# douban/fast_tffm

Measured on AMD Instinct MI355X. Metric: examples/sec (whole node), Criteo-shaped FM k=64, higher is better.
Workload: dtype fp32; 1 GPU; model=FM k=64, fp32 table + adagrad, hashed vocab 125000000 (125000000/GPU), global_batch=131072, seq_len=39, parallelism=single, lookahead=2, pool=16, rccl_world=1, comm_bytes_per_rank=0

## Files before the change

### fast_tffm_amd/csrc/hip/fm_common.h

```cpp
#pragma once
#include <hip/hip_runtime.h>
#include <hip/hip_bf16.h>
#include <cstdint>

namespace fm {

constexpr int kWave = 64;
constexpr int kBlock = 256;
constexpr int kWavesPerBlock = kBlock / kWave;

constexpr int kChunkSegMask = (1 << 30) - 1;
constexpr int kChunkFirst = 1 << 30;
constexpr unsigned kChunkSingle = 1u << 31;

constexpr int kDevErrSort = 1;
__device__ int g_fm_dev_error = 0;

enum LossType : int { kLossNone = 0, kLossMse = 1, kLossLogistic = 2 };
enum OptType : int { kOptAdagrad = 0, kOptFtrl = 1, kOptSgd = 2 };
enum DType : int { kF32 = 0, kBF16 = 1, kFP8 = 2 };

struct fp8e4m3 { uint8_t bits; };
constexpr float kFp8Max = 448.f;

// ... 237 lines not shown
  if constexpr (StateBf16<TV>::v) {
    uint16_t* p = reinterpret_cast<uint16_t*>(s) + off;
    uint32_t b[EPL];
#pragma unroll
    for (int k = 0; k < EPL; k += 4) {
      if (seed) {
        const uint32_t r = sr_hash(seed, row, col + (uint32_t)k);
#pragma unroll
        for (int i = 0; i < 4; ++i) b[k + i] = f32_to_bf16_bits_sr(o[k + i], sr_word(r, i));
      } else {
#pragma unroll
        for (int i = 0; i < 4; ++i) b[k + i] = f32_to_bf16_bits(o[k + i]);
      }
    }
    if constexpr (EPL % 8 == 0) {
#pragma unroll
      for (int k = 0; k < EPL; k += 8)
        *reinterpret_cast<uint4*>(p + k) = make_uint4(b[k] | (b[k + 1] << 16), b[k + 2] | (b[k + 3] << 16),
                                                      b[k + 4] | (b[k + 5] << 16), b[k + 6] | (b[k + 7] << 16));
    } else {
#pragma unroll
      for (int k = 0; k < EPL; k += 4)
        *reinterpret_cast<uint2*>(p + k) = make_uint2(b[k] | (b[k + 1] << 16), b[k + 2] | (b[k + 3] << 16));
    }
  } else {
    float* p = reinterpret_cast<float*>(s) + off;
#pragma unroll
    for (int k = 0; k < EPL; k += 4) *reinterpret_cast<float4*>(p + k) = make_float4(o[k], o[k + 1], o[k + 2], o[k + 3]);
  }
}
constexpr uint32_t kSrSalt0 = 0x68e31da4u, kSrSalt1 = 0xb5297a4du;

template <typename TV>
__device__ inline float row_scale(const float* w, long long row, long long w_stride) {
  if constexpr (Frag<TV>::kScaled) return w[row * w_stride + 1];
  return 1.f;
}

constexpr int kFp8Norm = 2;
template <int LPR>
__device__ inline float fp8_norm2(int u, float s, bool tact) {
  float q[4];
  Frag<fp8e4m3>::cvt(u, q);
  float p = tact ? __fmaf_rn(q[0], q[0], __fmaf_rn(q[1], q[1], __fmaf_rn(q[2], q[2], q[3] * q[3]))) : 0.f;
  p = group_sum<LPR>(p);
  return p * (s * s);
}

template <int LPR, typename TV>
__device__ inline void store_row(TV* lane_ptr, const float (&o)[Frag<TV>::N], float* w, long long row,
                                 long long w_stride, int t, bool tact, uint32_t sr_seed = 0) {
  using F = Frag<TV>;
  const uint32_t col = (uint32_t)(t * F::N);
  if constexpr (F::kScaled) {
    float m = 0.f;
#pragma unroll
    for (int k = 0; k < F::N; ++k) m = fmaxf(m, fabsf(o[k]));
    m = group_max<LPR>(m);
    const float s = fp8_row_scale(m);
    const float inv = 1.f / s;
    float q[F::N];
#pragma unroll
    for (int k = 0; k < F::N; ++k) q[k] = fminf(fmaxf(o[k] * inv, -kFp8Max), kFp8Max);
    int u = 0;
    if (tact) u = sr_seed ? F::store_sr(lane_ptr, q, sr_seed, (uint32_t)row, col) : F::store(lane_ptr, q);
    const float n2 = fp8_norm2<LPR>(u, s, tact);
    if (t == 0) {
      w[row * w_stride + 1] = s;
      w[row * w_stride + kFp8Norm] = n2;
    }
  } else {
    if (tact) {
      if (sr_seed) F::store_sr(lane_ptr, o, sr_seed, (uint32_t)row, col);
      else F::store(lane_ptr, o);
    }
  }
}

template <int LPR>
__device__ inline void store_row_fp8x8(fp8e4m3* lane_ptr, const float (&o)[8], float* w, long long row,
                                       long long w_stride, int t, bool tact, uint32_t sr_seed) {
  using F = Frag<fp8e4m3>;
  float m = 0.f;
#pragma unroll
  for (int k = 0; k < 8; ++k) m = fmaxf(m, fabsf(o[k]));
  m = group_max<LPR>(m);
  const float s = fp8_row_scale(m);
  const float inv = 1.f / s;
  float qa[4], qb[4];
#pragma unroll
  for (int k = 0; k < 4; ++k) {
    qa[k] = fminf(fmaxf(o[k] * inv, -kFp8Max), kFp8Max);
    qb[k] = fminf(fmaxf(o[k + 4] * inv, -kFp8Max), kFp8Max);
  }
  const uint32_t col = (uint32_t)(t * 8);
  int ua = 0, ub = 0;
  if (tact) {
    ua = sr_seed ? F::pack_sr(qa, sr_seed, (uint32_t)row, col) : F::pack(qa);
    ub = sr_seed ? F::pack_sr(qb, sr_seed, (uint32_t)row, col + 4) : F::pack(qb);
    *reinterpret_cast<uint2*>(lane_ptr) = make_uint2((uint32_t)ua, (uint32_t)ub);
  }
  float pa[4], pb[4];
  F::cvt(ua, pa);
  F::cvt(ub, pb);
  float na = tact ? __fmaf_rn(pa[0], pa[0], __fmaf_rn(pa[1], pa[1], __fmaf_rn(pa[2], pa[2], pa[3] * pa[3]))) : 0.f;
  float nb = tact ? __fmaf_rn(pb[0], pb[0], __fmaf_rn(pb[1], pb[1], __fmaf_rn(pb[2], pb[2], pb[3] * pb[3]))) : 0.f;
  na = group_sum<LPR>(na);
  nb = group_sum<LPR>(nb);
  const float n2 = (na + nb) * (s * s);
  if (t == 0) {
    w[row * w_stride + 1] = s;
    w[row * w_stride + kFp8Norm] = n2;
  }
}

#ifndef FM_FP8_WIDE
#define FM_FP8_WIDE 1
#endif

template <typename TV, int EPL>
__device__ inline void frag_load(const TV* p, float (&o)[EPL]) {
  if constexpr (EPL == Frag<TV>::N) {
    Frag<TV>::load(p, o);
  } else {
    static_assert(std::is_same<TV, fp8e4m3>::value && EPL == 8, "wide rows: fp8, 8 values per lane");
    const uint2 u = *reinterpret_cast<const uint2*>(p);
    float lo[4], hi[4];
    Frag<TV>::cvt((int)u.x, lo);
    Frag<TV>::cvt((int)u.y, hi);
#pragma unroll
    for (int k = 0; k < 4; ++k) {
      o[k] = lo[k];
      o[k + 4] = hi[k];
    }
  }
}
template <int LPR, typename TV, int EPL>
__device__ inline void store_row_e(TV* lane_ptr, const float (&o)[EPL], float* w, long long row, long long w_stride,
                                   int t, bool tact, uint32_t sr) {
  if constexpr (EPL == Frag<TV>::N) store_row<LPR, TV>(lane_ptr, o, w, row, w_stride, t, tact, sr);
  else store_row_fp8x8<LPR>(lane_ptr, o, w, row, w_stride, t, tact, sr);
}

__device__ inline uint32_t sr_step_seed(const int* counter) {
  return counter ? (sr_hash((uint32_t)*counter, 0x5bd1e995u, 0x1b873593u) | 1u) : 0u;
}

template <int LPR>
__device__ inline float across_groups_sum(float v) {
#pragma unroll
  for (int o = LPR; o < kWave; o <<= 1) v += __shfl_xor(v, o, kWave);
  return v;
}

__device__ inline float softplus_neg_abs(float p) {
  return log1pf(__expf(-fabsf(p)));
}

__device__ inline float sigmoidf(float p) { return 1.f / (1.f + __expf(-p)); }

struct OptParams {
  int type;
  float lr;
  float l1, l2;
  float beta;
};

struct SelfRows {
  int u0, u1;
  long long base;
  const int* keys;
  const int* excl;
  const void* v; long long v_stride;
  float* w; long long w_stride;
  __device__ inline bool has(int u) const { return u >= u0 && u < u1; }
  __device__ inline bool exclusive(int u) const { return excl == nullptr || excl[u - u0] != 0; }
  __device__ inline long long row(int u) const { return (long long)keys[u] - base; }
};

__device__ inline void opt_step(const OptParams& o, float g, float& p, float& s0, float& s1) {
  if (o.type == kOptAdagrad) {
    s0 += g * g;
    p -= o.lr * g * rsqrtf(s0);
  } else if (o.type == kOptFtrl) {
    const float n_new = s0 + g * g;
    const float sq_old = sqrtf(s0), sq_new = sqrtf(n_new);
    s1 += g - (sq_new - sq_old) / o.lr * p;
    s0 = n_new;
    const float quad = (o.beta + sq_new) / o.lr + 2.f * o.l2;
    p = fabsf(s1) > o.l1 ? (copysignf(o.l1, s1) - s1) / quad : 0.f;
  } else {
    p -= o.lr * g;
  }
}

template <typename TV>
__device__ inline void opt_step_tv(const OptParams& o, float g, float& p, float& s0, float& s1) {
  if constexpr (FM_FP8_FAST_EPI && StateBf16<TV>::v) {
    if (o.type == kOptFtrl) {
      const float ilr = __builtin_amdgcn_rcpf(o.lr);
      const float n_new = __builtin_fmaf(g, g, s0);
      const float sq_old = __builtin_amdgcn_sqrtf(s0), sq_new = __builtin_amdgcn_sqrtf(n_new);
      s1 += __builtin_fmaf(-((sq_new - sq_old) * ilr), p, g);
      s0 = n_new;
      const float quad = __builtin_fmaf(o.beta + sq_new, ilr, 2.f * o.l2);
      p = fabsf(s1) > o.l1 ? (copysignf(o.l1, s1) - s1) * __builtin_amdgcn_rcpf(quad) : 0.f;
      return;
    }
    if (o.type == kOptAdagrad) {
      s0 = __builtin_fmaf(g, g, s0);
      p = __builtin_fmaf(-(o.lr * g), __builtin_amdgcn_rsqf(s0), p);
      return;
    }
  }
  opt_step(o, g, p, s0, s1);
}

template <typename TV, int N>
__device__ inline void opt_step_row(const OptParams& o, const float (&g)[N], float (&p)[N], float (&s0)[N],
                                    float (&s1)[N]) {
  if (o.type == kOptFtrl) {
    OptParams f = o;
    f.type = kOptFtrl;
#pragma unroll
    for (int k = 0; k < N; ++k) opt_step_tv<TV>(f, g[k], p[k], s0[k], s1[k]);
  } else if (o.type == kOptAdagrad) {
    OptParams f = o;
    f.type = kOptAdagrad;
#pragma unroll
    for (int k = 0; k < N; ++k) opt_step_tv<TV>(f, g[k], p[k], s0[k], s1[k]);
  } else {
#pragma unroll
    for (int k = 0; k < N; ++k) p[k] -= o.lr * g[k];
  }
}

inline int next_pow2(int x) { int p = 1; while (p < x) p <<= 1; return p; }

inline int lanes_per_row(int Kp, int dtype) {
  const int epl = 4;
  return next_pow2((Kp + epl - 1) / epl);
}

inline int lds_for_wg_per_cu(int n, int static_lds) {
  static const int cu_lds = [] {
    int dev = 0, v = 0;
    (void)hipGetDevice(&dev);
    if (hipDeviceGetAttribute(&v, hipDeviceAttributeMaxSharedMemoryPerMultiprocessor, dev) != hipSuccess || v <= 0)
      v = 160 * 1024;
    return v;
  }();
  const int per = cu_lds / (n + 1) + 1024 - static_lds;
  return per > 0 && (per + static_lds) * n <= cu_lds ? per : 0;
}

inline int fill_grid(long long work_groups, int groups_per_block, int cap = 8192) {
  long long blocks = (work_groups + groups_per_block - 1) / groups_per_block;
  if (blocks < 1) blocks = 1;
  if (blocks > cap) blocks = cap;
  return (int)blocks;
}

#define FM_DISPATCH_LPR(LPR_VAL, KERNEL, TV, GRID, SHM, STREAM, ARGS)                                   \
  switch (LPR_VAL) {                                                                                     \
    case 1: hipLaunchKernelGGL((KERNEL<1, TV>), dim3(GRID), dim3(kBlock), SHM, STREAM, ARGS); break;     \
    case 2: hipLaunchKernelGGL((KERNEL<2, TV>), dim3(GRID), dim3(kBlock), SHM, STREAM, ARGS); break;     \
    case 4: hipLaunchKernelGGL((KERNEL<4, TV>), dim3(GRID), dim3(kBlock), SHM, STREAM, ARGS); break;     \
    case 8: hipLaunchKernelGGL((KERNEL<8, TV>), dim3(GRID), dim3(kBlock), SHM, STREAM, ARGS); break;     \
    case 16: hipLaunchKernelGGL((KERNEL<16, TV>), dim3(GRID), dim3(kBlock), SHM, STREAM, ARGS); break;   \
    case 32: hipLaunchKernelGGL((KERNEL<32, TV>), dim3(GRID), dim3(kBlock), SHM, STREAM, ARGS); break;   \
    case 64: hipLaunchKernelGGL((KERNEL<64, TV>), dim3(GRID), dim3(kBlock), SHM, STREAM, ARGS); break;   \
    default: return -1;                                                                                  \
  }

#define FM_DISPATCH_WIDE_LPR(LPR_VAL, KERNEL, TV, GRID, SHM, STREAM, ARGS)                              \
  switch (LPR_VAL) {                                                                                     \
    case 4: hipLaunchKernelGGL((KERNEL<4, TV>), dim3(GRID), dim3(kBlock), SHM, STREAM, ARGS); break;     \
    case 8: hipLaunchKernelGGL((KERNEL<8, TV>), dim3(GRID), dim3(kBlock), SHM, STREAM, ARGS); break;     \
    case 16: hipLaunchKernelGGL((KERNEL<16, TV>), dim3(GRID), dim3(kBlock), SHM, STREAM, ARGS); break;   \
    case 32: hipLaunchKernelGGL((KERNEL<32, TV>), dim3(GRID), dim3(kBlock), SHM, STREAM, ARGS); break;   \
    case 64: hipLaunchKernelGGL((KERNEL<64, TV>), dim3(GRID), dim3(kBlock), SHM, STREAM, ARGS); break;   \
    default: return -1;                                                                                  \
  }

#define FM_DISPATCH_TV(DTYPE, M, LPR_VAL, KERNEL, GRID, SHM, STREAM, ARGS)   \
  if ((DTYPE) == kBF16) {                                                   \
    M(LPR_VAL, KERNEL, __hip_bfloat16, GRID, SHM, STREAM, ARGS)             \
  } else if ((DTYPE) == kFP8) {                                             \
    M(LPR_VAL, KERNEL, fp8e4m3, GRID, SHM, STREAM, ARGS)                    \
  } else {                                                                  \
    M(LPR_VAL, KERNEL, float, GRID, SHM, STREAM, ARGS)                      \
  }
#define FM_DISPATCH_WIDE(DTYPE, LPR_VAL, KERNEL, GRID, SHM, STREAM, ARGS) \
  FM_DISPATCH_TV(DTYPE, FM_DISPATCH_WIDE_LPR, LPR_VAL, KERNEL, GRID, SHM, STREAM, ARGS)
#define FM_DISPATCH_SHM(DTYPE, LPR_VAL, KERNEL, GRID, SHM, STREAM, ARGS) \
  FM_DISPATCH_TV(DTYPE, FM_DISPATCH_LPR, LPR_VAL, KERNEL, GRID, SHM, STREAM, ARGS)
#define FM_DISPATCH(DTYPE, LPR_VAL, KERNEL, GRID, STREAM, ARGS) \
  FM_DISPATCH_SHM(DTYPE, LPR_VAL, KERNEL, GRID, 0, STREAM, ARGS)

}
```

### fast_tffm_amd/csrc/hip/fm_fwd.hip

```cpp
#include "fm_common.h"

namespace fm {

struct FwdArgs {
  int B;
  const int* offsets;
  const int* rows;
  const float* vals;
  const void* v;
  long long v_stride;
  const float* w;
  long long w_stride;
  int Kp;
  const float* labels;
  const float* weights;
  int loss_type;
  float grad_scale;
  float* pred;
  void* r1;
  float* dpred;
  float* loss_partial;
  float* reg_partial;
  const float* bias;
  SelfRows self;
  const int* seg_idx;
  const int* seg_keys;
  int seg_shift;
  int max_feats;
};

__device__ inline int seg_lookup(const FwdArgs& a, int k) {
  const int b = (int)((uint32_t)k >> a.seg_shift);
  int s = a.seg_idx[b];
  const int e = a.seg_idx[b + 1];
  while (s + 1 < e && a.seg_keys[s] != k) ++s;
  return s;
}

#ifndef FM_FWD_PREFETCH
#define FM_FWD_PREFETCH 1
#endif
#ifndef FM_FWD_SPECIALIZE
#define FM_FWD_SPECIALIZE 1
#endif
constexpr int kSelfBit = (int)0x80000000u;
template <int G>
struct FwdUnroll {
  static constexpr int v = ((40 + G - 1) / G) > 12 ? 12 : ((40 + G - 1) / G);
};

template <int LPR, typename TV>
constexpr int fwd_min_waves() {
  return LPR >= 32 ? 4 : 1;
}
#ifndef FM_FWD_LOCAL_W16
#define FM_FWD_LOCAL_W16 7
#endif
#ifndef FM_FWD_UNR16
#define FM_FWD_UNR16 2
#endif
#ifndef FM_FWD_LOCAL_W32
#define FM_FWD_LOCAL_W32 4
#endif
#ifndef FM_FWD_UNR32
#define FM_FWD_UNR32 12
#endif
#ifndef FM_FWD_LOCAL_W32_FP8
#define FM_FWD_LOCAL_W32_FP8 7
#endif
#ifndef FM_FWD_UNR32_FP8
#define FM_FWD_UNR32_FP8 4
#endif
#ifndef FM_FWD_LOCAL_W4
#define FM_FWD_LOCAL_W4 4
#endif
#ifndef FM_FWD_UNR4
#define FM_FWD_UNR4 5
#endif
#ifndef FM_FWD_UNR16_SH
#define FM_FWD_UNR16_SH 10
#endif
#ifndef FM_FWD_SH_W16
#define FM_FWD_SH_W16 4
#endif
template <typename TV>
constexpr bool fwd_is_bf16() { return std::is_same<TV, __hip_bfloat16>::value; }
template <int LPR, typename TV, bool SH = false>
constexpr int fwd_local_min_waves() {
  return LPR == 4 && fwd_is_bf16<TV>() && FM_FWD_LOCAL_W4 > 0 ? FM_FWD_LOCAL_W4
         : LPR == 16 ? (SH && !Frag<TV>::kScaled ? FM_FWD_SH_W16 : FM_FWD_LOCAL_W16)
         : LPR == 32 ? (Frag<TV>::kScaled ? FM_FWD_LOCAL_W32_FP8 : FM_FWD_LOCAL_W32)
                     : fwd_min_waves<LPR, TV>();
}
template <int LPR, typename TV, bool SH = false>
constexpr int fwd_unroll() {
  return LPR == 16 && SH && !Frag<TV>::kScaled ? FM_FWD_UNR16_SH
         : LPR == 4 && fwd_is_bf16<TV>() && FM_FWD_UNR4 > 0 ? FM_FWD_UNR4
         : LPR == 16 ? FM_FWD_UNR16
         : LPR == 32 ? (Frag<TV>::kScaled ? FM_FWD_UNR32_FP8 : FM_FWD_UNR32)
                     : FwdUnroll<kWave / LPR>::v;
}

template <int LPR, typename TV, bool SH>
__device__ __forceinline__ void fwd_body(const FwdArgs& a) {
  using F = Frag<TV>;
  constexpr int EPL = F::N;
  constexpr int G = kWave / LPR;
  constexpr int UNR = fwd_unroll<LPR, TV, SH>();
  constexpr bool kRaw = F::kScaled;
  constexpr bool kNorm = F::kScaled;
  const int lane = threadIdx.x & (kWave - 1);
  const int g = lane / LPR, t = lane % LPR;
  const int nv = a.Kp / EPL;
  const bool tact = t < nv;
  const int tE = tact ? t : nv - 1;
  const float tmask = tact ? 1.f : 0.f;
  const uint32_t coff = (uint32_t)(tE * EPL * (int)sizeof(TV));
  const char* vbytes = reinterpret_cast<const char*>(a.v) + coff;
  const uint32_t vsb = (uint32_t)(a.v_stride * (long long)sizeof(TV));
  const bool self_on = SH && a.self.u1 > a.self.u0;
  const uint32_t tsb = self_on ? (uint32_t)(a.self.v_stride * (long long)sizeof(TV)) : vsb;
  const uint64_t wbase = reinterpret_cast<uint64_t>(a.v) + coff;
  const uint64_t sbase = self_on ? reinterpret_cast<uint64_t>(a.self.v) + coff : wbase;
  const int wave = blockIdx.x * kWavesPerBlock + (threadIdx.x >> 6);
  const int nwaves = gridDim.x * kWavesPerBlock;
  const bool want_reg = a.reg_partial != nullptr;
  const bool self_key = SH && self_on && a.seg_idx != nullptr;
  const int self_kmin = self_key ? a.self.keys[a.self.u0] : 0;
  const int self_kmax = self_key ? a.self.keys[a.self.u1 - 1] : -1;
  const int wv = threadIdx.x >> 6;

  float loss_acc = 0.f, regv_acc = 0.f, regw_acc = 0.f;
  constexpr bool kPrefetch = FM_FWD_PREFETCH;
  auto pairs = [&](int base, int m, int& row, float& x) {
    row = 0;
    x = 0.f;
    if (lane < m) {
      row = a.rows[base + lane];
      x = a.vals ? a.vals[base + lane] : 1.f;
    }
  };
  int s = 0, e = 0, sn = 0, en = 0;
  int p_row = 0;
  float p_x = 0.f;
  if (wave < a.B) {
    s = a.offsets[wave];
    e = a.offsets[wave + 1];
    if (kPrefetch) pairs(s, min(kWave, e - s), p_row, p_x);
  }
  if (wave + nwaves < a.B) {
    sn = a.offsets[wave + nwaves];
    en = a.offsets[wave + nwaves + 1];
  }
  for (int i = wave; i < a.B; i += nwaves) {
    int n_row = 0;
    float n_x = 0.f;
    if (kPrefetch) pairs(sn, i + nwaves < a.B ? min(kWave, en - sn) : 0, n_row, n_x);
    int snn = 0, enn = 0;
    if (i + 2 * nwaves < a.B) {
      snn = a.offsets[i + 2 * nwaves];
      enn = a.offsets[i + 2 * nwaves + 1];
    }
    float y_pre = 0.f, wt_pre = 1.f;
    if (kPrefetch && a.loss_type != kLossNone && lane == 0) {
      y_pre = a.labels[i];
      if (a.weights) wt_pre = a.weights[i];
    }
    float s1[EPL], s2[EPL];
#pragma unroll
    for (int k = 0; k < EPL; ++k) { s1[k] = 0.f; s2[k] = 0.f; }
    float lin = 0.f, rv = 0.f, rw = 0.f;
    float s2n = 0.f;
    for (int base = s; base < e; base += kWave) {
      const int m = min(kWave, e - base);
      int my_row = 0;
      float my_x = 0.f, my_w = 0.f, my_s = 1.f, my_n2 = 0.f;
      uint32_t my_t = 0;
      if (kPrefetch && base == s) {
        my_row = p_row;
        my_x = p_x;
      } else {
        pairs(base, m, my_row, my_x);
      }
      if constexpr (!SH) {
        if (lane < m) {
          if constexpr (kNorm) {
            const float4 wr = *reinterpret_cast<const float4*>(a.w + (uint64_t)(uint32_t)my_row * 4u);
            my_w = wr.x;
            my_s = wr.y;
            my_n2 = wr.z;
          } else {
            my_w = a.w[(long long)my_row * a.w_stride];
          }
        }
      } else {
        if (lane < m) {
          const int key = my_row;
          const bool own_key = self_key && key >= self_kmin && key <= self_kmax;
          if (a.seg_idx && !own_key) my_row = seg_lookup(a, key);
          const bool own = own_key || (self_on && !self_key && a.self.has(my_row));
          const long long r = own ? (own_key ? (long long)key - a.self.base : a.self.row(my_row)) : my_row;
          my_t = (uint32_t)r | (own ? 0x80000000u : 0u);
          const uint64_t wp = reinterpret_cast<uint64_t>(own ? a.self.w + r * a.self.w_stride : a.w + r * a.w_stride);
          if constexpr (kNorm) {
            const gf4 wr = *gptr<gf4>(wp);
            my_w = wr.x;
            my_s = wr.y;
            my_n2 = wr.z;
          } else {
            my_w = *gptr<float>(wp);
          }
        }
        const uint32_t t0 = (uint32_t)__builtin_amdgcn_readfirstlane((int)my_t);
        if (lane >= m) my_t = t0;
      }

      for (int q = 0; q < m; q += G * UNR) {
        float fr[UNR][EPL], fx[UNR], fs[UNR];
        int fraw[kRaw ? UNR : 1];
#pragma unroll
        for (int u = 0; u < UNR; ++u) {
          const int f = q + u * G + g;
          const int fb = (f & (kWave - 1)) << 2;
          const float x = __int_as_float(__builtin_amdgcn_ds_bpermute(fb, __float_as_int(my_x)));
          fx[u] = f < m ? x : 0.f;
          if constexpr (SH) {
            const uint32_t tr = (uint32_t)__builtin_amdgcn_ds_bpermute(fb, (int)my_t);
            const bool own = (tr >> 31) != 0;
            const uint64_t pr = (own ? sbase : wbase) + (uint64_t)(tr & 0x7fffffffu) * (own ? tsb : vsb);
            if constexpr (kRaw) fraw[u] = *gptr<int>(pr);
            else F::load_g(pr, fr[u]);
          } else {
            const int row = __builtin_amdgcn_ds_bpermute(fb, my_row);
            const char* rp = vbytes + (uint64_t)(uint32_t)row * vsb;
            if constexpr (kRaw) fraw[u] = *reinterpret_cast<const int*>(rp);
            else F::load(reinterpret_cast<const TV*>(rp), fr[u]);
          }
          if constexpr (F::kScaled) fs[u] = __int_as_float(__builtin_amdgcn_ds_bpermute(fb, __float_as_int(my_s)));
        }
#pragma unroll
        for (int u = 0; u < UNR; ++u) {
          float (&fv)[EPL] = fr[u];
          if constexpr (kRaw) F::cvt_scaled(fraw[u], fs[u], fv);
          const float xm = fx[u] * tmask;
#pragma unroll
          for (int k = 0; k < EPL; ++k) {
            const float xv = xm * fv[k];
            s1[k] += xv;
            if constexpr (!kNorm) s2[k] += xv * xv;
          }
          if (!kNorm && want_reg) {
            const float ok = (q + u * G + g) < m ? 1.f : 0.f;
#pragma unroll
            for (int k = 0; k < EPL; ++k) rv += ok * tmask * fv[k] * fv[k];
          }
        }
      }
      lin += my_x * my_w;
      if (want_reg) rw += my_w * my_w;
      if constexpr (kNorm) {
        s2n += my_x * my_x * my_n2;
        if (want_reg && lane < m) rv += my_n2;
      }
    }
    float part = 0.f;
#pragma unroll
    for (int k = 0; k < EPL; ++k) {
      s1[k] = across_groups_sum<LPR>(s1[k]);
      s2[k] = across_groups_sum<LPR>(s2[k]);
      part += s1[k] * s1[k] - s2[k];
    }
    part = group_sum<LPR>(part);
    if constexpr (kNorm) part -= group_sum<kWave>(s2n);
    lin = group_sum<kWave>(lin);
    const float pred = lin + 0.5f * part + (a.bias ? a.bias[0] : 0.f);
    if (a.r1 != nullptr && g == 0 && tact) store_r1<TV, EPL>(a.r1, (long long)i * a.Kp + t * EPL, s1);
    if (want_reg) {
      rv = group_sum<kWave>(rv);
      rw = group_sum<kWave>(rw);
      regv_acc += rv;
      regw_acc += rw;
    }
    float l = 0.f, d = 0.f;
    if (a.loss_type != kLossNone && lane == 0) {
      const float y = kPrefetch ? y_pre : a.labels[i];
      const float wt = kPrefetch ? wt_pre : (a.weights ? a.weights[i] : 1.f);
      if (a.loss_type == kLossMse) {
        const float diff = pred - y;
        l = wt * diff * diff;
        d = 2.f * wt * diff;
      } else {
        l = wt * (fmaxf(pred, 0.f) - pred * y + softplus_neg_abs(pred));
        d = wt * (sigmoidf(pred) - y);
      }
    }
    if (lane == 0) {
      a.pred[i] = pred;
      if (a.loss_type != kLossNone) {
        loss_acc += l;
        if (a.dpred) a.dpred[i] = d * a.grad_scale;
      }
    }
    s = sn; e = en; sn = snn; en = enn;
    p_row = n_row; p_x = n_x;
  }
  if (a.loss_partial == nullptr && a.reg_partial == nullptr) return;
  __shared__ float red[3][kWavesPerBlock];
  if (lane == 0) {
    red[0][wv] = loss_acc;
    red[1][wv] = regv_acc;
    red[2][wv] = regw_acc;
  }
  __syncthreads();
  if (threadIdx.x == 0) {
    float l = 0.f, r0 = 0.f, r1v = 0.f;
    for (int k = 0; k < kWavesPerBlock; ++k) { l += red[0][k]; r0 += red[1][k]; r1v += red[2][k]; }
    if (a.loss_partial) a.loss_partial[blockIdx.x] = l;
    if (a.reg_partial) { a.reg_partial[2 * blockIdx.x] = r0; a.reg_partial[2 * blockIdx.x + 1] = r1v; }
  }
}

template <int LPR, typename TV>
__global__ __launch_bounds__(kBlock) __attribute__((amdgpu_waves_per_eu(fwd_local_min_waves<LPR, TV>())))
void fm_fwd_kernel(FwdArgs a) {
  fwd_body<LPR, TV, false>(a);
}

template <int LPR, typename TV>
__global__ __launch_bounds__(kBlock) __attribute__((amdgpu_waves_per_eu(fwd_local_min_waves<LPR, TV, true>())))
void fm_fwd_shard_kernel(FwdArgs a) {
  fwd_body<LPR, TV, true>(a);
}

#ifndef FM_WITH_MFMA
#define FM_WITH_MFMA 0
#endif
#if FM_WITH_MFMA
#include "fm_fwd_mfma.hip"
#endif

__global__ __launch_bounds__(kBlock) void csr_rows_kernel(int B, const int* offsets, int* ex_of_occ, int slot_bits) {
  const int lane = threadIdx.x & (kWave - 1);
  const int ngroups = (B + kWave - 1) / kWave;
  const int nwaves = gridDim.x * kWavesPerBlock;
  for (int g = blockIdx.x * kWavesPerBlock + (threadIdx.x >> 6); g < ngroups; g += nwaves) {
    const int i0 = g * kWave;
    const int n = min(kWave, B - i0);
    const int o = offsets[i0 + min(lane, n)];
    const int s = __shfl(o, 0);
    const int e = offsets[i0 + n];
    for (int base = s; base < e; base += kWave) {
      const int p = base + lane;
      int k = 0;
#pragma unroll
      for (int step = kWave / 2; step > 0; step >>= 1) {
        const int c = k + step;
        if (__shfl(o, c) <= p) k = c;
      }
      const int ok = __shfl(o, k);
      if (p < e) {
        const int ex = i0 + k;
        ex_of_occ[p] = slot_bits > 0 ? (ex << slot_bits) | (p - ok) : ex;
      }
    }
  }
}

static bool g_fwd_mfma = FM_WITH_MFMA;
bool fwd_mfma_enabled() { return g_fwd_mfma; }
void set_fwd_mfma(bool on) { g_fwd_mfma = FM_WITH_MFMA && on; }

int fwd_grid(int B) { return fill_grid(B, kWavesPerBlock, 4096); }

int launch_fwd(const FwdArgs& a, int dtype, int grid, hipStream_t st) {
  if (a.B <= 0) return 0;
  const int lpr = lanes_per_row(a.Kp, dtype);
  if (dtype == kFP8) {
    auto aligned = [](const float* w, long long ws) { return ((uintptr_t)w & 15) == 0 && ws % 4 == 0; };
    if (!aligned(a.w, a.w_stride) || (a.self.u1 > a.self.u0 && !aligned(a.self.w, a.self.w_stride))) return -7;
  }
  const bool table_rows = dtype != kFP8 || a.w_stride == 4;
#if FM_WITH_MFMA
  if (fwd_mfma_enabled() && dtype == kFP8 && a.Kp == kMfRowB && a.v_stride == kMfRowB && !a.vals && table_rows &&
      a.self.u1 <= a.self.u0 && !a.seg_idx && a.max_feats > 0 && a.max_feats * kMfT <= kMfMaxRows) {
    hipLaunchKernelGGL(fm_fwd_mfma_fp8_kernel, dim3(grid), dim3(kBlock), 0, st, a);
    return (int)hipGetLastError();
  }
#endif

  if (a.self.u1 > a.self.u0 || a.seg_idx || !FM_FWD_SPECIALIZE || !table_rows) {
    FM_DISPATCH(dtype, lpr, fm_fwd_shard_kernel, grid, st, a);
  } else {
    FM_DISPATCH(dtype, lpr, fm_fwd_kernel, grid, st, a);
  }
  return (int)hipGetLastError();
}

int launch_csr_rows(int B, const int* offsets, int* ex_of_occ, int slot_bits, hipStream_t st) {
  if (B <= 0) return 0;
  hipLaunchKernelGGL(csr_rows_kernel, dim3(fill_grid((B + kWave - 1) / kWave, kWavesPerBlock, 4096)), dim3(kBlock), 0, st, B,
                     offsets, ex_of_occ, slot_bits);
  return (int)hipGetLastError();
}

}
```

### fast_tffm_amd/csrc/hip/module.hip

```cpp
#include <pybind11/pybind11.h>
#include <pybind11/stl.h>
#include <stdexcept>
#include <string>
#include "fm_common.h"

namespace py = pybind11;

#ifndef FM_HIP_MODULE
#define FM_HIP_MODULE _fm_hip
#endif
using u64 = std::uintptr_t;

#include "fm_bwd.hip"
#include "fm_fwd.hip"
#include "fm_explain.hip"
#include "fm_topk.hip"
#include "dedup.hip"
#include "metric_common.hip"
#include "auc.hip"
#include "isotonic.hip"
#include "gauc.hip"
#include "shard.hip"
#include "init.hip"
#include "ckpt.hip"
#include "parse.hip"
#include "batch_gather.hip"
#include "feeder.hip"

namespace {

template <typename T> T* P(u64 p) { return reinterpret_cast<T*>(p); }
hipStream_t S(u64 s) { return reinterpret_cast<hipStream_t>(s); }

void check(int code, const char* what) {
  if (code != 0) {
    std::string msg = std::string(what) + " failed: ";
    msg += code > 0 ? hipGetErrorString(static_cast<hipError_t>(code)) : ("code " + std::to_string(code));
    throw std::runtime_error(msg);
  }
}

fm::SelfRows self_rows(const std::vector<long long>& f) {
  fm::SelfRows r{};
  if (f.empty()) return r;
  if (f.size() != 9) throw std::invalid_argument("self_rows: [u0, u1, base, keys, excl, v, v_stride, w, w_stride]");
  if (f[1] > f[0] && (!f[3] || !f[5] || !f[7])) throw std::runtime_error("self rows need keys and the table");
  r.u0 = (int)f[0]; r.u1 = (int)(f[1] > f[0] ? f[1] : f[0]); r.base = f[2];
  r.keys = P<const int>((u64)f[3]); r.excl = P<const int>((u64)f[4]);
  r.v = P<const void>((u64)f[5]); r.v_stride = f[6]; r.w = P<float>((u64)f[7]); r.w_stride = f[8];
  return r;
}

fm::OptParams opt_params(int type, float lr, float l1, float l2, float beta) {
  fm::OptParams o;
  o.type = type; o.lr = lr; o.l1 = l1; o.l2 = l2; o.beta = beta;
  return o;
}

}

#ifndef FM_BUILD_HASH
#define FM_BUILD_HASH "unhashed"
#endif
extern "C" __attribute__((used, visibility("default"))) const char fm_build_hash_marker[] = "FMBUILDHASH:" FM_BUILD_HASH;

PYBIND11_MODULE(FM_HIP_MODULE, m) {
  m.doc() = "gfx950 HIP kernels for fast_tffm_amd (FM forward/backward/optimizer, dedup, sharding)";
  m.attr("ARCH") = "gfx950";
  m.attr("BUILD_HASH") = FM_BUILD_HASH;
  m.attr("MAX_CH") = fm::kMaxCH;

  m.def("fwd_grid", &fm::fwd_grid, py::arg("B"));
  m.def("fwd_mfma_enabled", &fm::fwd_mfma_enabled);
  m.def("set_fwd_mfma", &fm::set_fwd_mfma, py::arg("on"));
#if FM_MF_PROF
  m.def("mf_prof", [] {
    unsigned long long h[8] = {};
    hipDeviceSynchronize();
    hipMemcpyFromSymbol(h, HIP_SYMBOL(fm::g_mf_prof), sizeof(h));
    const unsigned long long z[8] = {};
    hipMemcpyToSymbol(HIP_SYMBOL(fm::g_mf_prof), z, sizeof(z));
    return std::vector<unsigned long long>(h, h + 8);
  });
#endif
  m.def("lanes_per_row", &fm::lanes_per_row, py::arg("Kp"), py::arg("dtype"));

  m.def(
      "fwd",
      [](int B, u64 offsets, u64 rows, u64 vals, u64 v, long long v_stride, u64 w, long long w_stride, int Kp,
         int dtype, u64 labels, u64 weights, int loss_type, float grad_scale, u64 pred, u64 r1, u64 dpred,
         u64 loss_partial, u64 reg_partial, int grid, u64 stream, u64 bias, const std::vector<long long>& self,
         u64 seg_idx, u64 seg_keys, int seg_shift, int max_feats) {
        fm::FwdArgs a{};
        a.max_feats = max_feats;
        a.seg_idx = P<const int>(seg_idx); a.seg_keys = P<const int>(seg_keys); a.seg_shift = seg_shift;
        if (a.seg_idx && (!a.seg_keys || seg_shift < 0 || seg_shift > 31))
          throw std::invalid_argument("fm_fwd: segment lookup needs the sorted keys and a shift in [0, 31]");
        a.self = self_rows(self);
        a.B = B; a.offsets = P<const int>(offsets); a.rows = P<const int>(rows);
        a.vals = P<const float>(vals); a.v = P<const void>(v); a.v_stride = v_stride;
        a.w = P<const float>(w); a.w_stride = w_stride; a.Kp = Kp;
        a.labels = P<const float>(labels); a.weights = P<const float>(weights);
        a.loss_type = loss_type; a.grad_scale = grad_scale; a.pred = P<float>(pred);
        a.r1 = P<void>(r1); a.dpred = P<float>(dpred); a.loss_partial = P<float>(loss_partial);
        a.reg_partial = P<float>(reg_partial); a.bias = P<const float>(bias);
        check(fm::launch_fwd(a, dtype, grid, S(stream)), "fm_fwd");
      },
      py::arg("B"), py::arg("offsets"), py::arg("rows"), py::arg("vals"), py::arg("v"), py::arg("v_stride"),
      py::arg("w"), py::arg("w_stride"), py::arg("Kp"), py::arg("dtype"), py::arg("labels"), py::arg("weights"),
      py::arg("loss_type"), py::arg("grad_scale"), py::arg("pred"), py::arg("r1"), py::arg("dpred"),
      py::arg("loss_partial"), py::arg("reg_partial"), py::arg("grid"), py::arg("stream"), py::arg("bias") = 0,
      py::arg("self_rows") = std::vector<long long>{}, py::arg("seg_idx") = 0, py::arg("seg_keys") = 0,
      py::arg("seg_shift") = 0, py::arg("max_feats") = -1);

  m.def(
      "explain",
      [](int B, u64 offsets, u64 rows, u64 vals, u64 v, long long v_stride, u64 w, long long w_stride, int Kp,
         int dtype, u64 bias, u64 contrib, u64 pred, u64 stream) {
        fm::ExplainArgs a{};
        a.B = B; a.offsets = P<const int>(offsets); a.rows = P<const int>(rows); a.vals = P<const float>(vals);
        a.v = P<const void>(v); a.v_stride = v_stride; a.w = P<const float>(w); a.w_stride = w_stride; a.Kp = Kp;
        a.bias = P<const float>(bias); a.contrib = P<float>(contrib); a.pred = P<float>(pred);
        check(fm::launch_explain(a, dtype, S(stream)), "fm_explain");
      },
      py::arg("B"), py::arg("offsets"), py::arg("rows"), py::arg("vals"), py::arg("v"), py::arg("v_stride"),
      py::arg("w"), py::arg("w_stride"), py::arg("Kp"), py::arg("dtype"), py::arg("bias"), py::arg("contrib"),
      py::arg("pred"), py::arg("stream"));
  m.def(
      "importance",
      [](int U, u64 contrib, u64 perm, u64 seg_start, u64 count, u64 sum_abs, u64 sum, u64 stream) {
        fm::ImportanceArgs a{};
        a.U = U; a.contrib = P<const float>(contrib); a.perm = P<const int>(perm);
        a.seg_start = P<const int>(seg_start); a.count = P<int>(count); a.sum_abs = P<double>(sum_abs);
        a.sum = P<double>(sum);
        check(fm::launch_importance(a, S(stream)), "fm_importance");
      },
      py::arg("U"), py::arg("contrib"), py::arg("perm"), py::arg("seg_start"), py::arg("count"), py::arg("sum_abs"),
      py::arg("sum"), py::arg("stream"));

  m.def(
      "topk_plan",
      [](long long nq, long long nc, int k) {
        const fm::topk::Plan p = fm::topk::plan(nq, nc, k);
        return py::make_tuple(p.slab, p.parts);
      },
      py::arg("nq"), py::arg("nc"), py::arg("k"));
  m.def("topk_workspace_bytes", &fm::topk_workspace_bytes, py::arg("nq"), py::arg("nc"), py::arg("k"));
  m.def(
      "topk",
      [](long long nq, long long nc, int Kp, int k, u64 q, long long q_stride, u64 c, long long c_stride, u64 qb,
         u64 cb, u64 ws, size_t ws_bytes, u64 idx, u64 score, u64 stream) {
        if ((long long)ws_bytes < fm::topk_workspace_bytes(nq, nc, k)) throw std::runtime_error("topk: workspace too small");
        fm::TopkArgs a{};
        a.nq = nq; a.nc = nc; a.Kp = Kp; a.k = k; a.Q = P<const float>(q); a.q_stride = q_stride;
        a.C = P<const float>(c); a.c_stride = c_stride; a.qb = P<const float>(qb); a.cb = P<const float>(cb);
        a.ws = P<unsigned long long>(ws); a.idx = P<int>(idx); a.score = P<float>(score);
        check(fm::launch_topk(a, S(stream)), "fm_topk");
      },
      py::arg("nq"), py::arg("nc"), py::arg("Kp"), py::arg("k"), py::arg("q"), py::arg("q_stride"), py::arg("c"),
      py::arg("c_stride"), py::arg("qb"), py::arg("cb"), py::arg("ws"), py::arg("ws_bytes"), py::arg("idx"),
      py::arg("score"), py::arg("stream"));

  m.def(
      "seg_index",
      [](int n_max, u64 uniq, u64 counts, int shift, int nb, u64 idx, u64 stream) {
        check(fm::launch_seg_index(n_max, P<const uint32_t>(uniq), P<const int>(counts), shift, nb, P<int>(idx),
                                   S(stream)),
              "seg_index");
      },
      py::arg("n_max"), py::arg("uniq"), py::arg("counts"), py::arg("shift"), py::arg("nb"), py::arg("idx"),
      py::arg("stream"));

  m.def(
      "bwd",
      [](int mode, u64 counts, u64 chunk_start, u64 chunk_seg, u64 chunk_key, u64 seg_start, u64 seg_chunk, u64 uniq,
         u64 sorted_ex, int ex_shift, u64 sorted_x, u64 dpred, u64 r1, int Kp, u64 v, long long v_stride, u64 w,
         long long w_stride, u64 s0v, u64 s1v, long long s_stride, u64 s0w, u64 s1w, float reg_v, float reg_w,
         int opt_type, float lr, float l1, float l2, float beta, u64 grad_out, long long g_stride, u64 partial,
         u64 big_list, u64 big_count, u64 multi, int nex, int dtype,
         long long max_chunks, long long max_unique, u64 stream, int g_wcol, int g_bf16, u64 sr_counter,
         int counters_ready, u64 seg_bounds, int piece, int n_owners,
         const std::vector<long long>& self) {
        fm::BwdArgs a{};
        a.self = self_rows(self);
        if (a.self.u1 > a.self.u0 && a.self.keys != P<const int>(uniq))
          throw std::runtime_error("fm_bwd: self-row keys must be the dedup's unique keys");
        if (a.self.u1 > a.self.u0 && (mode != 1 || !s0v || !s0w))
          throw std::runtime_error("fm_bwd: self rows are an EMIT-mode path and need the table's optimizer state");
        a.counters_ready = counters_ready;
        a.seg_bounds = P<const int>(seg_bounds); a.piece = piece; a.n_owners = n_owners;
        a.sr_counter = P<const int>(sr_counter);
        a.mode = mode; a.counts = P<const int>(counts); a.chunk_start = P<const int>(chunk_start);
        a.chunk_seg = P<const int>(chunk_seg); a.chunk_key = P<const int>(chunk_key);
        a.seg_start = P<const int>(seg_start);
        a.seg_chunk = P<const int>(seg_chunk); a.uniq = P<const int>(uniq);
        a.sorted_ex = P<const int>(sorted_ex); a.ex_shift = ex_shift; a.sorted_x = P<const float>(sorted_x);
        a.dpred = P<const float>(dpred); a.r1 = P<const void>(r1); a.Kp = Kp;
        a.v = P<void>(v); a.v_stride = v_stride; a.w = P<float>(w); a.w_stride = w_stride;
        a.s0v = P<void>(s0v); a.s1v = P<void>(s1v); a.s_stride = s_stride; a.s0w = P<float>(s0w);
        a.s1w = P<float>(s1w); a.reg_v = reg_v; a.reg_w = reg_w;
        a.opt = opt_params(opt_type, lr, l1, l2, beta);
        a.grad_out = P<float>(grad_out); a.g_stride = g_stride; a.g_wcol = g_wcol < 0 ? Kp : g_wcol;
        a.g_bf16 = g_bf16; a.partial = P<float>(partial);
        a.big_list = P<int>(big_list); a.big_count = P<int>(big_count); a.multi = P<int>(multi);
        a.counts_rw = P<int>(counts);
        a.nex = nex;
        check(fm::launch_bwd(a, dtype, max_chunks, max_unique, S(stream)), "fm_bwd");
      },
      py::arg("mode"), py::arg("counts"), py::arg("chunk_start"), py::arg("chunk_seg"), py::arg("chunk_key"),
      py::arg("seg_start"),
      py::arg("seg_chunk"), py::arg("uniq"), py::arg("sorted_ex"), py::arg("ex_shift"), py::arg("sorted_x"), py::arg("dpred"),
      py::arg("r1"), py::arg("Kp"), py::arg("v"), py::arg("v_stride"), py::arg("w"), py::arg("w_stride"),
      py::arg("s0v"), py::arg("s1v"), py::arg("s_stride"), py::arg("s0w"), py::arg("s1w"), py::arg("reg_v"),
      py::arg("reg_w"), py::arg("opt_type"), py::arg("lr"), py::arg("l1"), py::arg("l2"), py::arg("beta"),
      py::arg("grad_out"), py::arg("g_stride"), py::arg("partial"), py::arg("big_list"), py::arg("big_count"),
      py::arg("multi"), py::arg("nex"), py::arg("dtype"),
      py::arg("max_chunks"), py::arg("max_unique"), py::arg("stream"), py::arg("g_wcol") = -1,
      py::arg("g_bf16") = 0, py::arg("sr_counter") = 0, py::arg("counters_ready") = 0, py::arg("seg_bounds") = 0,
      py::arg("piece") = -1, py::arg("n_owners") = 0,
      py::arg("self_rows") = std::vector<long long>{});

  m.def("dedup_workspace_bytes", &fm::dedup_workspace_bytes, py::arg("n"));
  m.def("set_sort_algo", &fm::set_sort_algo, py::arg("in_tree"));
  m.def("sort_algo", &fm::sort_algo);
  m.def(
      "radix_sort",
      [](u64 keys, u64 vals, u64 kout, u64 vout, int n, int end_bit, u64 ws, size_t ws_bytes, u64 stream) {
        check(fm::launch_radix_sort(P<const uint32_t>(keys), P<const int>(vals), P<uint32_t>(kout), P<int>(vout), n,
                                    end_bit, P<void>(ws), ws_bytes, S(stream)),
              "radix_sort");
        if (n <= 0) return;
        int err = 0;
        check((int)hipMemcpyAsync(&err, fm::radix_sort_error(P<void>(ws), n), sizeof(int), hipMemcpyDeviceToHost,
                                  S(stream)),
              "radix_sort error word");
        check((int)hipStreamSynchronize(S(stream)), "radix_sort sync");
        if (err) throw std::runtime_error("radix_sort: look-back spin bound hit");
      },
      py::arg("keys"), py::arg("vals"), py::arg("kout"), py::arg("vout"), py::arg("n"), py::arg("end_bit"),
      py::arg("ws"), py::arg("ws_bytes"), py::arg("stream"));
  m.def("radix_sort_ws_bytes", &fm::radix_sort_ws_bytes, py::arg("n"));
  m.def("bwd_wide_launches", &fm::bwd_wide_launches);
  m.def("set_sort_spin_cap", &fm::set_sort_spin_cap, py::arg("cap"));
  m.def(
      "device_errors",
      [](bool clear) {
        int v = 0;
        check((int)hipDeviceSynchronize(), "device_errors sync");
        check((int)hipMemcpyFromSymbol(&v, HIP_SYMBOL(fm::g_fm_dev_error), sizeof(int)), "device_errors read");
        if (clear && v) {
          const int z = 0;
          check((int)hipMemcpyToSymbol(HIP_SYMBOL(fm::g_fm_dev_error), &z, sizeof(int)), "device_errors clear");
        }
        return v;
      },
      py::arg("clear") = false);
  m.def(
      "dedup",
      [](int n, int end_bit, int CH, u64 keys, u64 payload, u64 skeys, u64 spay, u64 uniq, u64 seg_start,
         u64 seg_chunk, u64 chunk_start, u64 chunk_seg, u64 chunk_key, u64 counts, u64 inv, u64 ex_of_occ,
         u64 sorted_ex, u64 vals, u64 sorted_x, int payload_is_ex, int ex_shift, u64 offsets, u64 ws,
         size_t ws_bytes, u64 stream, u64 ids, int kW, int kRps, int gen_codes, int B) {
        if (CH < 1 || CH > fm::kMaxCH) throw std::invalid_argument("CH must be in [1, MAX_CH]");
        fm::DedupArgs a;
        a.n = n; a.end_bit = end_bit; a.CH = CH; a.keys = P<const uint32_t>(keys);
        a.payload = P<const int>(payload); a.skeys = P<uint32_t>(skeys); a.spay = P<int>(spay);
// ... 403 lines not shown
```

Measured before the change: 223.8 million examples/s.

## Specialize fp32 forward: DPP/permlane reductions, implicit x=1, batched per-lane loss epilogue

For fp32 tables, the forward kernel now does its cross-lane sums with DPP and permlane16/32 swap butterflies in place of ds_bpermute shuffles. It adds a no-values variant that drops the per-feature x broadcast and multiply when vals is null. Predictions are parked one per lane and flushed in groups of 64, so label loads, loss math and pred/dpred stores run across 64 lanes at once instead of serially on lane 0. A probe kernel is added to check that the new reduction primitives are correct. The changes add template variants and a serial readlane accumulation of the loss, and they rely on MI355X-specific permlane builtins.

```diff
diff --git a/fast_tffm_amd/csrc/hip/fm_common.h b/fast_tffm_amd/csrc/hip/fm_common.h
--- a/fast_tffm_amd/csrc/hip/fm_common.h
+++ b/fast_tffm_amd/csrc/hip/fm_common.h
@@ -413,6 +413,42 @@
   for (int o = LPR; o < kWave; o <<= 1) v += __shfl_xor(v, o, kWave);
   return v;
 }
+
+template <int O>
+__device__ inline float xor_add(float v) {
+  static_assert(O == 1 || O == 2 || O == 4 || O == 8 || O == 16 || O == 32, "xor butterfly step");
+  if constexpr (O == 32 || O == 16) {
+    const uint32_t u = __float_as_uint(v);
+    if constexpr (O == 32) {
+      const auto r = __builtin_amdgcn_permlane32_swap(u, u, false, false);
+      return __uint_as_float(r[0]) + __uint_as_float(r[1]);
+    } else {
+      const auto r = __builtin_amdgcn_permlane16_swap(u, u, false, false);
+      return __uint_as_float(r[0]) + __uint_as_float(r[1]);
+    }
+  } else if constexpr (O == 4) {
+    return v + __shfl_xor(v, 4, kWave);
+  } else {
+    constexpr int ctrl = O == 8 ? 0x128 : O == 2 ? 0x4E : 0xB1;
+    return v + __int_as_float(__builtin_amdgcn_update_dpp(0, __float_as_int(v), ctrl, 0xf, 0xf, false));
+  }
+}
+
+template <int O>
+__device__ inline float xor_add_down(float v) {
+  if constexpr (O >= 1) return xor_add_down<O / 2>(xor_add<O>(v));
+  else return v;
+}
+template <int O>
+__device__ inline float xor_add_up(float v) {
+  if constexpr (O < kWave) return xor_add_up<O * 2>(xor_add<O>(v));
+  else return v;
+}
+
+template <int WIDTH>
+__device__ inline float group_sum_x(float v) { return xor_add_down<WIDTH / 2>(v); }
+template <int LPR>
+__device__ inline float across_groups_sum_x(float v) { return xor_add_up<LPR>(v); }
 
 __device__ inline float softplus_neg_abs(float p) {
   return log1pf(__expf(-fabsf(p)));
diff --git a/fast_tffm_amd/csrc/hip/fm_fwd.hip b/fast_tffm_amd/csrc/hip/fm_fwd.hip
--- a/fast_tffm_amd/csrc/hip/fm_fwd.hip
+++ b/fast_tffm_amd/csrc/hip/fm_fwd.hip
@@ -102,8 +102,39 @@
 }
 
 template <int LPR, typename TV, bool SH>
+constexpr bool fwd_x_sums() { return std::is_same<TV, float>::value; }
+template <int LPR, typename TV, bool SH>
+constexpr bool fwd_park_loss() { return std::is_same<TV, float>::value; }
+template <int LPR, typename TV, bool SH>
+constexpr bool fwd_nox() { return std::is_same<TV, float>::value; }
+
+template <bool X, int WIDTH>
+__device__ __forceinline__ float fwd_group_sum(float v) {
+  if constexpr (X) return group_sum_x<WIDTH>(v);
+  else return group_sum<WIDTH>(v);
+}
+template <bool X, int LPR>
+__device__ __forceinline__ float fwd_across_sum(float v) {
+  if constexpr (X) return across_groups_sum_x<LPR>(v);
+  else return across_groups_sum<LPR>(v);
+}
+
+__device__ __forceinline__ void fwd_loss(int loss_type, float pred, float y, float wt, float& l, float& d) {
+  if (loss_type == kLossMse) {
+    const float diff = pred - y;
+    l = wt * diff * diff;
+    d = 2.f * wt * diff;
+  } else {
+    l = wt * (fmaxf(pred, 0.f) - pred * y + softplus_neg_abs(pred));
+    d = wt * (sigmoidf(pred) - y);
+  }
+}
+
+template <int LPR, typename TV, bool SH, bool NOX>
 __device__ __forceinline__ void fwd_body(const FwdArgs& a) {
   using F = Frag<TV>;
+  constexpr bool kX = fwd_x_sums<LPR, TV, SH>();
+  constexpr bool kPark = fwd_park_loss<LPR, TV, SH>();
   constexpr int EPL = F::N;
   constexpr int G = kWave / LPR;
   constexpr int UNR = fwd_unroll<LPR, TV, SH>();
@@ -137,8 +168,24 @@
     x = 0.f;
     if (lane < m) {
       row = a.rows[base + lane];
-      x = a.vals ? a.vals[base + lane] : 1.f;
-    }
+      x = !NOX && a.vals ? a.vals[base + lane] : 1.f;
+    }
+  };
+  float park = 0.f;
+  int n_done = 0;
+  auto flush = [&](int n0, int cnt) {
+    float l = 0.f;
+    if (lane < cnt) {
+      const int ii = wave + (n0 + lane) * nwaves;
+      a.pred[ii] = park;
+      if (a.loss_type != kLossNone) {
+        float d;
+        fwd_loss(a.loss_type, park, a.labels[ii], a.weights ? a.weights[ii] : 1.f, l, d);
+        if (a.dpred) a.dpred[ii] = d * a.grad_scale;
+      }
+    }
+    if (a.loss_type != kLossNone)
+      for (int j = 0; j < cnt; ++j) loss_acc += __int_as_float(__builtin_amdgcn_readlane(__float_as_int(l), j));
   };
   int s = 0, e = 0, sn = 0, en = 0;
   int p_row = 0;
@@ -162,7 +209,7 @@
       enn = a.offsets[i + 2 * nwaves + 1];
     }
     float y_pre = 0.f, wt_pre = 1.f;
-    if (kPrefetch && a.loss_type != kLossNone && lane == 0) {
+    if (!kPark && kPrefetch && a.loss_type != kLossNone && lane == 0) {
       y_pre = a.labels[i];
       if (a.weights) wt_pre = a.weights[i];
     }
@@ -216,14 +263,16 @@
       }
 
       for (int q = 0; q < m; q += G * UNR) {
-        float fr[UNR][EPL], fx[UNR], fs[UNR];
+        float fr[UNR][EPL], fx[NOX ? 1 : UNR], fs[UNR];
         int fraw[kRaw ? UNR : 1];
 #pragma unroll
         for (int u = 0; u < UNR; ++u) {
           const int f = q + u * G + g;
           const int fb = (f & (kWave - 1)) << 2;
-          const float x = __int_as_float(__builtin_amdgcn_ds_bpermute(fb, __float_as_int(my_x)));
-          fx[u] = f < m ? x : 0.f;
+          if constexpr (!NOX) {
+            const float x = __int_as_float(__builtin_amdgcn_ds_bpermute(fb, __float_as_int(my_x)));
+            fx[u] = f < m ? x : 0.f;
+          }
           if constexpr (SH) {
             const uint32_t tr = (uint32_t)__builtin_amdgcn_ds_bpermute(fb, (int)my_t);
             const bool own = (tr >> 31) != 0;
@@ -242,12 +291,22 @@
         for (int u = 0; u < UNR; ++u) {
           float (&fv)[EPL] = fr[u];
           if constexpr (kRaw) F::cvt_scaled(fraw[u], fs[u], fv);
-          const float xm = fx[u] * tmask;
-#pragma unroll
-          for (int k = 0; k < EPL; ++k) {
-            const float xv = xm * fv[k];
-            s1[k] += xv;
-            if constexpr (!kNorm) s2[k] += xv * xv;
+          if constexpr (NOX) {
+            const bool on = tact && (q + u * G + g) < m;
+#pragma unroll
+            for (int k = 0; k < EPL; ++k) {
+              const float xv = on ? fv[k] : 0.f;
+              s1[k] += xv;
+              if constexpr (!kNorm) s2[k] = __builtin_fmaf(xv, xv, s2[k]);
+            }
+          } else {
+            const float xm = fx[u] * tmask;
+#pragma unroll
+            for (int k = 0; k < EPL; ++k) {
+              const float xv = xm * fv[k];
+              s1[k] += xv;
+              if constexpr (!kNorm) s2[k] += xv * xv;
+            }
           }
           if (!kNorm && want_reg) {
             const float ok = (q + u * G + g) < m ? 1.f : 0.f;
@@ -266,43 +325,46 @@
     float part = 0.f;
 #pragma unroll
     for (int k = 0; k < EPL; ++k) {
-      s1[k] = across_groups_sum<LPR>(s1[k]);
-      s2[k] = across_groups_sum<LPR>(s2[k]);
+      s1[k] = fwd_across_sum<kX, LPR>(s1[k]);
+      s2[k] = fwd_across_sum<kX, LPR>(s2[k]);
       part += s1[k] * s1[k] - s2[k];
     }
-    part = group_sum<LPR>(part);
-    if constexpr (kNorm) part -= group_sum<kWave>(s2n);
-    lin = group_sum<kWave>(lin);
+    part = fwd_group_sum<kX, LPR>(part);
+    if constexpr (kNorm) part -= fwd_group_sum<kX, kWave>(s2n);
+    lin = fwd_group_sum<kX, kWave>(lin);
     const float pred = lin + 0.5f * part + (a.bias ? a.bias[0] : 0.f);
     if (a.r1 != nullptr && g == 0 && tact) store_r1<TV, EPL>(a.r1, (long long)i * a.Kp + t * EPL, s1);
     if (want_reg) {
-      rv = group_sum<kWave>(rv);
-      rw = group_sum<kWave>(rw);
+      rv = fwd_group_sum<kX, kWave>(rv);
+      rw = fwd_group_sum<kX, kWave>(rw);
       regv_acc += rv;
       regw_acc += rw;
     }
-    float l = 0.f, d = 0.f;
-    if (a.loss_type != kLossNone && lane == 0) {
-      const float y = kPrefetch ? y_pre : a.labels[i];
-      const float wt = kPrefetch ? wt_pre : (a.weights ? a.weights[i] : 1.f);
-      if (a.loss_type == kLossMse) {
-        const float diff = pred - y;
-        l = wt * diff * diff;
-        d = 2.f * wt * diff;
-      } else {
-        l = wt * (fmaxf(pred, 0.f) - pred * y + softplus_neg_abs(pred));
-        d = wt * (sigmoidf(pred) - y);
-      }
-    }
-    if (lane == 0) {
-      a.pred[i] = pred;
-      if (a.loss_type != kLossNone) {
-        loss_acc += l;
-        if (a.dpred) a.dpred[i] = d * a.grad_scale;
+    if constexpr (kPark) {
+      if (lane == (n_done & (kWave - 1))) park = pred;
+      ++n_done;
+      if ((n_done & (kWave - 1)) == 0) flush(n_done - kWave, kWave);
+    } else {
+      float l = 0.f, d = 0.f;
+      if (a.loss_type != kLossNone && lane == 0) {
+        const float y = kPrefetch ? y_pre : a.labels[i];
+        const float wt = kPrefetch ? wt_pre : (a.weights ? a.weights[i] : 1.f);
+        fwd_loss(a.loss_type, pred, y, wt, l, d);
+      }
+      if (lane == 0) {
+        a.pred[i] = pred;
+        if (a.loss_type != kLossNone) {
+          loss_acc += l;
+          if (a.dpred) a.dpred[i] = d * a.grad_scale;
+        }
       }
     }
     s = sn; e = en; sn = snn; en = enn;
     p_row = n_row; p_x = n_x;
+  }
+  if constexpr (kPark) {
+    const int n_all = __builtin_amdgcn_readfirstlane(n_done);
+    if (n_all & (kWave - 1)) flush(n_all & ~(kWave - 1), n_all & (kWave - 1));
   }
   if (a.loss_partial == nullptr && a.reg_partial == nullptr) return;
   __shared__ float red[3][kWavesPerBlock];
@@ -323,13 +385,23 @@
 template <int LPR, typename TV>
 __global__ __launch_bounds__(kBlock) __attribute__((amdgpu_waves_per_eu(fwd_local_min_waves<LPR, TV>())))
 void fm_fwd_kernel(FwdArgs a) {
-  fwd_body<LPR, TV, false>(a);
+  fwd_body<LPR, TV, false, false>(a);
+}
+template <int LPR, typename TV>
+__global__ __launch_bounds__(kBlock) __attribute__((amdgpu_waves_per_eu(fwd_local_min_waves<LPR, TV>())))
+void fm_fwd_kernel_nox(FwdArgs a) {
+  fwd_body<LPR, TV, false, fwd_nox<LPR, TV, false>()>(a);
 }
 
 template <int LPR, typename TV>
 __global__ __launch_bounds__(kBlock) __attribute__((amdgpu_waves_per_eu(fwd_local_min_waves<LPR, TV, true>())))
 void fm_fwd_shard_kernel(FwdArgs a) {
-  fwd_body<LPR, TV, true>(a);
+  fwd_body<LPR, TV, true, false>(a);
+}
+template <int LPR, typename TV>
+__global__ __launch_bounds__(kBlock) __attribute__((amdgpu_waves_per_eu(fwd_local_min_waves<LPR, TV, true>())))
+void fm_fwd_shard_kernel_nox(FwdArgs a) {
+  fwd_body<LPR, TV, true, fwd_nox<LPR, TV, true>()>(a);
 }
 
 #ifndef FM_WITH_MFMA
@@ -388,11 +460,33 @@
   }
 #endif
 
+  const bool nox = a.vals == nullptr && dtype == kF32;
   if (a.self.u1 > a.self.u0 || a.seg_idx || !FM_FWD_SPECIALIZE || !table_rows) {
-    FM_DISPATCH(dtype, lpr, fm_fwd_shard_kernel, grid, st, a);
+    if (nox) { FM_DISPATCH_LPR(lpr, fm_fwd_shard_kernel_nox, float, grid, 0, st, a); }
+    else { FM_DISPATCH(dtype, lpr, fm_fwd_shard_kernel, grid, st, a); }
   } else {
-    FM_DISPATCH(dtype, lpr, fm_fwd_kernel, grid, st, a);
-  }
+    if (nox) { FM_DISPATCH_LPR(lpr, fm_fwd_kernel_nox, float, grid, 0, st, a); }
+    else { FM_DISPATCH(dtype, lpr, fm_fwd_kernel, grid, st, a); }
+  }
+  return (int)hipGetLastError();
+}
+
+template <int I>
+__device__ inline void reduce_probe_store(float v, float* out, int n, int idx) {
+  constexpr int W = 2 << I, L = 1 << I;
+  out[(0 * 6 + I) * (long long)n + idx] = group_sum<W>(v);
+  out[(1 * 6 + I) * (long long)n + idx] = group_sum_x<W>(v);
+  out[(2 * 6 + I) * (long long)n + idx] = across_groups_sum<L>(v);
+  out[(3 * 6 + I) * (long long)n + idx] = across_groups_sum_x<L>(v);
+  if constexpr (I < 5) reduce_probe_store<I + 1>(v, out, n, idx);
+}
+__global__ __launch_bounds__(kWave) void fwd_reduce_probe_kernel(const float* x, float* out, int n) {
+  const int idx = blockIdx.x * kWave + threadIdx.x;
+  reduce_probe_store<0>(x[idx], out, n, idx);
+}
+int launch_fwd_reduce_probe(const float* x, int waves, float* out, hipStream_t st) {
+  if (waves <= 0) return 0;
+  hipLaunchKernelGGL(fwd_reduce_probe_kernel, dim3(waves), dim3(kWave), 0, st, x, out, waves * kWave);
   return (int)hipGetLastError();
 }
 
diff --git a/fast_tffm_amd/csrc/hip/module.hip b/fast_tffm_amd/csrc/hip/module.hip
--- a/fast_tffm_amd/csrc/hip/module.hip
+++ b/fast_tffm_amd/csrc/hip/module.hip
@@ -112,6 +112,13 @@
       py::arg("loss_partial"), py::arg("reg_partial"), py::arg("grid"), py::arg("stream"), py::arg("bias") = 0,
       py::arg("self_rows") = std::vector<long long>{}, py::arg("seg_idx") = 0, py::arg("seg_keys") = 0,
       py::arg("seg_shift") = 0, py::arg("max_feats") = -1);
+
+  m.def(
+      "fwd_reduce_probe",
+      [](u64 x, int waves, u64 out, u64 stream) {
+        check(fm::launch_fwd_reduce_probe(P<const float>(x), waves, P<float>(out), S(stream)), "fwd_reduce_probe");
+      },
+      py::arg("x"), py::arg("waves"), py::arg("out"), py::arg("stream"));
 
   m.def(
       "explain",
```

After: 226.7 million examples/s, median of 6. 1.3% higher.
